# ChuhanZhou/News_Recommendation_Model

Hardware: AMD Instinct MI355X
Metric: train impressions/sec (higher is better)
Workload: dtype f32

## Files before the change

news_recommendation_model_amd/csrc/frontend.hip:

```cpp
#include <algorithm>
#include "common.hpp"
#include "frontend.hpp"

namespace nrm {

template <typename XT>
__device__ __forceinline__ int row_index(const XT* xr, int col, int limit, int* err) {
    const int i = (int)xr[col];
    if (i < 0 || i >= limit) { *err = 1; return i < 0 ? 0 : limit - 1; }
    return i;
}

constexpr int FE_MAXSUB = 16;
constexpr int FE_HDR = 6 + FE_MAXSUB;
struct RowHeaders {
    int* idx;
    float* sen;
};

template <typename XT>
__device__ __forceinline__ void stage_headers(const FrontendParams& p, int xcols, int* err, const XT* __restrict__ x, int r_lo, int nr,
                                              const RowHeaders& hd, int nthreads) {
    const int P = p.P, NS = p.n_sub;
    const int c_cat = 4 + P, c_sub = c_cat + 1, c_sen = c_sub + NS, c_typ = c_sen + 3;
    const int items = 9 + NS;
    for (int i = threadIdx.x; i < nr * items; i += nthreads) {
        const int r = i / items, k = i - r * items;
        const XT* xr = x + (size_t)(r_lo + r) * xcols;
        if (k < 4) {
            const int lim = k == 0 ? p.n_year : k == 1 ? p.n_month : k == 2 ? p.n_day : p.n_hour;
            hd.idx[r * FE_HDR + k] = row_index(xr, k, lim, err);
        } else if (k == 4) {
            hd.idx[r * FE_HDR + 4] = row_index(xr, c_cat, p.n_cat, err);
        } else if (k == 5) {
            hd.idx[r * FE_HDR + 5] = row_index(xr, c_typ, p.n_type, err);
        } else if (k < 6 + NS) {
            hd.idx[r * FE_HDR + k] = row_index(xr, c_sub + (k - 6), p.n_cat, err);
        } else {
            hd.sen[r * 4 + (k - 6 - NS)] = (float)xr[c_sen + (k - 6 - NS)];
        }
    }
}

constexpr int FWD_ROWS = 8;
constexpr int FE_THREADS = 256;

template <typename XT>
__global__ __launch_bounds__(FE_THREADS) void frontend_fwd_kernel(const FrontendParams p, const XT* __restrict__ x, int nrows) {
    __shared__ int h_idx[FWD_ROWS * FE_HDR];
    __shared__ float h_sen[FWD_ROWS * 4];
    const int r_lo = blockIdx.x * FWD_ROWS, nr = min(FWD_ROWS, nrows - r_lo);
    const RowHeaders hd = {h_idx, h_sen};
    stage_headers(p, p.xcols, p.err, x, r_lo, nr, hd, FE_THREADS);
    __syncthreads();
    const int P = p.P, NS = p.n_sub;
    const int c_beh = 4 + P + 1 + NS + 3 + 1;
    const int e0 = p.e0, e1 = p.e1, e2 = p.e2, e3 = p.e3;
    const int width = e0 + e1 + e2 + e3 + (p.behaviour ? 2 : 0);
    const float inv_ns = 1.0f / (float)NS;
    float* lab = p.lab + (size_t)r_lo * p.ldlab;
    for (int i = threadIdx.x; i < nr * p.ldlab; i += FE_THREADS) {
        const int r = i / p.ldlab, c = i - r * p.ldlab;
        const int* hi = h_idx + r * FE_HDR;
        float v = 0.f;
        if (c < e0) {
            float sub = 0.f;
            for (int k = 0; k < NS; ++k) sub += p.cat_tab[(size_t)hi[6 + k] * e0 + c];
            v = p.cat_tab[(size_t)hi[4] * e0 + c] + sub * inv_ns;
        } else if (c < e0 + e1) {
            const int j = c - e0;
            const float pre = p.sen_b[j] + p.sen_w[j * 3] * h_sen[r * 4] + p.sen_w[j * 3 + 1] * h_sen[r * 4 + 1] + p.sen_w[j * 3 + 2] * h_sen[r * 4 + 2];
            v = fmaxf(pre, 0.f);
        } else if (c < e0 + e1 + e2) {
            v = p.type_tab[(size_t)hi[5] * e2 + (c - e0 - e1)];
        } else if (c < e0 + e1 + e2 + e3) {
            const int k = c - e0 - e1 - e2;
            v = p.year_tab[(size_t)hi[0] * e3 + k] + p.month_tab[(size_t)hi[1] * e3 + k] + p.day_tab[(size_t)hi[2] * e3 + k] + p.hour_tab[(size_t)hi[3] * e3 + k];
        } else if (c < width) {
            v = (float)x[(size_t)(r_lo + r) * p.xcols + c_beh + (c - (e0 + e1 + e2 + e3))];
        }
        lab[i] = v;
    }
    float* ti = p.ti + (size_t)r_lo * p.ldti;
    for (int i = threadIdx.x; i < nr * p.ldti; i += FE_THREADS) {
        const int r = i / p.ldti, c = i - r * p.ldti;
        ti[i] = c < P ? (float)x[(size_t)(r_lo + r) * p.xcols + 4 + c] : 0.f;
    }
}

constexpr int FE_ROWS = 32;
constexpr int FE_MAX_BLOCKS = 512;

template <typename XT>
__global__ __launch_bounds__(FE_THREADS) void frontend_bwd_kernel(const FrontendParams p, const XT* __restrict__ x,
                                                                 const float* __restrict__ dlab, int lddl, int nrows) {
    extern __shared__ float sm[];
    const int e0 = p.e0, e1 = p.e1, e2 = p.e2, e3 = p.e3;
    float* a_type = sm;
    float* a_year = a_type + p.n_type * e2;
    float* a_month = a_year + p.n_year * e3;
    float* a_day = a_month + p.n_month * e3;
    float* a_hour = a_day + p.n_day * e3;
    float* a_sen = a_hour + p.n_hour * e3;
    const int total = (int)(a_sen + e1 * 4 - sm);
    const RowHeaders hd = {reinterpret_cast<int*>(sm + total), sm + total + FE_ROWS * FE_HDR};
    for (int i = threadIdx.x; i < total; i += FE_THREADS) sm[i] = 0.f;
    int dummy = 0;
    const int NS = p.n_sub;
    const float inv_ns = 1.0f / (float)NS;
    const int small = e1 + e2 + e3;
    const int ngroups = (nrows + FE_ROWS - 1) / FE_ROWS;
    for (int grp = blockIdx.x; grp < ngroups; grp += gridDim.x) {
        const int r_lo = grp * FE_ROWS, nr = min(FE_ROWS, nrows - r_lo);
        __syncthreads();
        stage_headers(p, p.xcols, &dummy, x, r_lo, nr, hd, FE_THREADS);
        __syncthreads();
        const float* g0 = dlab + (size_t)r_lo * lddl;
        for (int i = threadIdx.x; i < (p.d_cat_tab ? nr * e0 : 0); i += FE_THREADS) {
            const int r = i / e0, c = i - r * e0;
            const int* hi = hd.idx + r * FE_HDR;
            const float gv = g0[(size_t)r * lddl + c];
            atomicAdd(p.d_cat_tab + (size_t)hi[4] * e0 + c, gv);
            const float gs = gv * inv_ns;
            for (int k = 0; k < NS; ++k) atomicAdd(p.d_cat_tab + (size_t)hi[6 + k] * e0 + c, gs);
        }
        for (int i = threadIdx.x; i < (p.d_type_tab ? nr * small : 0); i += FE_THREADS) {
            const int r = i / small, cs = i - r * small;
            const float gv = g0[(size_t)r * lddl + e0 + cs];
            const int* hi = hd.idx + r * FE_HDR;
            if (cs < e1) {
                const float s0 = hd.sen[r * 4], s1 = hd.sen[r * 4 + 1], s2 = hd.sen[r * 4 + 2];
                const float pre = p.sen_b[cs] + p.sen_w[cs * 3] * s0 + p.sen_w[cs * 3 + 1] * s1 + p.sen_w[cs * 3 + 2] * s2;
                if (pre > 0.f && gv != 0.f) {
                    atomicAdd(a_sen + cs * 4 + 0, gv * s0);
                    atomicAdd(a_sen + cs * 4 + 1, gv * s1);
                    atomicAdd(a_sen + cs * 4 + 2, gv * s2);
                    atomicAdd(a_sen + cs * 4 + 3, gv);
                }
            } else if (cs < e1 + e2) {
                atomicAdd(a_type + hi[5] * e2 + (cs - e1), gv);
            } else {
                const int k = cs - e1 - e2;
                atomicAdd(a_year + hi[0] * e3 + k, gv);
                atomicAdd(a_month + hi[1] * e3 + k, gv);
                atomicAdd(a_day + hi[2] * e3 + k, gv);
                atomicAdd(a_hour + hi[3] * e3 + k, gv);
            }
        }
    }
    __syncthreads();
    if (!p.d_type_tab) return;
    for (int i = threadIdx.x; i < p.n_type * e2; i += FE_THREADS) if (a_type[i] != 0.f) atomicAdd(p.d_type_tab + i, a_type[i]);
    for (int i = threadIdx.x; i < p.n_year * e3; i += FE_THREADS) if (a_year[i] != 0.f) atomicAdd(p.d_year_tab + i, a_year[i]);
    for (int i = threadIdx.x; i < p.n_month * e3; i += FE_THREADS) if (a_month[i] != 0.f) atomicAdd(p.d_month_tab + i, a_month[i]);
    for (int i = threadIdx.x; i < p.n_day * e3; i += FE_THREADS) if (a_day[i] != 0.f) atomicAdd(p.d_day_tab + i, a_day[i]);
    for (int i = threadIdx.x; i < p.n_hour * e3; i += FE_THREADS) if (a_hour[i] != 0.f) atomicAdd(p.d_hour_tab + i, a_hour[i]);
    for (int i = threadIdx.x; i < e1 * 4; i += FE_THREADS) {
        const float v = a_sen[i];
        if (v != 0.f) {
            const int j = i >> 2, w = i & 3;
            if (w < 3) atomicAdd(p.d_sen_w + j * 3 + w, v); else atomicAdd(p.d_sen_b + j, v);
        }
    }
}

static size_t bwd_lds_bytes(const FrontendParams& p) {
    return sizeof(float) * ((size_t)p.n_type * p.e2 + (size_t)(p.n_year + p.n_month + p.n_day + p.n_hour) * p.e3 + (size_t)p.e1 * 4 +
                            (size_t)FE_ROWS * (FE_HDR + 4));
}

hipError_t frontend_fwd_launch(const FrontendParams& p, const void* x, int x_is_f64, int nrows, hipStream_t st) {
    if (nrows <= 0) return hipSuccess;
    if (p.n_sub > FE_MAXSUB) return hipErrorInvalidValue;
    const dim3 grid((nrows + FWD_ROWS - 1) / FWD_ROWS);
    if (x_is_f64) hipLaunchKernelGGL(frontend_fwd_kernel<double>, grid, dim3(FE_THREADS), 0, st, p, (const double*)x, nrows);
    else          hipLaunchKernelGGL(frontend_fwd_kernel<float>, grid, dim3(FE_THREADS), 0, st, p, (const float*)x, nrows);
    return hipGetLastError();
}

hipError_t frontend_bwd_launch(const FrontendParams& p, const void* x, int x_is_f64, const float* dlab, int lddl,
                               int nrows, hipStream_t st) {
    if (nrows <= 0) return hipSuccess;
    const size_t shm = bwd_lds_bytes(p);
    if (shm > 160 * 1024 || p.n_sub > FE_MAXSUB) return hipErrorInvalidValue;
    const dim3 grid(std::min((nrows + FE_ROWS - 1) / FE_ROWS, FE_MAX_BLOCKS));
    if (x_is_f64) {
        if (shm > 64 * 1024) { hipError_t e = hipFuncSetAttribute((const void*)frontend_bwd_kernel<double>, hipFuncAttributeMaxDynamicSharedMemorySize, (int)shm); if (e != hipSuccess) return e; }
        hipLaunchKernelGGL(frontend_bwd_kernel<double>, grid, dim3(FE_THREADS), shm, st, p, (const double*)x, dlab, lddl, nrows);
    } else {
        if (shm > 64 * 1024) { hipError_t e = hipFuncSetAttribute((const void*)frontend_bwd_kernel<float>, hipFuncAttributeMaxDynamicSharedMemorySize, (int)shm); if (e != hipSuccess) return e; }
        hipLaunchKernelGGL(frontend_bwd_kernel<float>, grid, dim3(FE_THREADS), shm, st, p, (const float*)x, dlab, lddl, nrows);
    }
    return hipGetLastError();
}

constexpr int TB_THREADS = 512;
constexpr int TB_WAVES = TB_THREADS / 64;
constexpr int TB_ROWS = 32;
constexpr int TB_MAXT = 16;
constexpr int TB_MAXTILES = TB_WAVES * TB_MAXT;
constexpr int TB_WG_PER_CU = 2;
constexpr int TB_CB = 4;
constexpr int TB_RED_CELLS = 64, TB_RED_SLICES = 16;

struct TabTile {
    short hdr, ibase;
    short coff, ncol;
    int dst;
    short ldr, ldc;
};
struct TabSet { const void* x; const float* dlab; int nrows, xcols, lddl, nchunks; };
struct TabParams {
    FrontendParams p;
    TabSet set[2];
    int ntiles, tiles_per_wave, cells, ldb, chunks_per_wg;
    float* ws;
    TabTile tile[TB_MAXTILES];
};

__device__ __forceinline__ bool fe_finite(float v) { return fabsf(v) <= 3.402823466e+38f; }

template <typename XT, int NT>
__global__ __launch_bounds__(TB_THREADS, TB_WG_PER_CU * TB_WAVES / 4) void tab_grad_kernel(const TabParams q) {
    extern __shared__ float sm[];
    const FrontendParams& p = q.p;
    const int e0 = p.e0, e1 = p.e1, e2 = p.e2, e3 = p.e3;
    const int small = e1 + e2 + e3, ldb = q.ldb;
    float* s_b = sm;
    float* s_wb = s_b + TB_ROWS * ldb;
    float* s_sen = s_wb + 4 * e1;
    float* s_sa = s_sen + TB_ROWS * 4;
    int* s_idx = reinterpret_cast<int*>(s_sa + TB_ROWS * 4);
    const RowHeaders hd = {s_idx, s_sen};
    const int lane = threadIdx.x & 63, wave = __builtin_amdgcn_readfirstlane(threadIdx.x >> 6);
    const int li = lane & 15, lk = lane >> 4;

    for (int i = threadIdx.x; i < e1 * 4; i += TB_THREADS) s_wb[i] = (i & 3) < 3 ? p.sen_w[(i >> 2) * 3 + (i & 3)] : p.sen_b[i >> 2];

    const int t_lo = wave * q.tiles_per_wave;
    const int my_nt = max(0, min(q.tiles_per_wave, q.ntiles - t_lo));
    int t_desc[NT];
    f32x4 acc[NT];
#pragma unroll
    for (int t = 0; t < NT; ++t) {
        const TabTile& d = q.tile[min(t_lo + t, TB_MAXTILES - 1)];
        const int v = t < my_nt ? (d.hdr + 1) | (d.ibase << 3) | (d.coff << 18) : 1 | (0x7fff << 3);
        t_desc[t] = __builtin_amdgcn_readfirstlane(v);
        acc[t] = f32x4{0.f, 0.f, 0.f, 0.f};
    }

    int dummy = 0;
    const int nchunks = q.set[0].nchunks + q.set[1].nchunks;
    const int ch_lo = blockIdx.x * q.chunks_per_wg, ch_hi = min(nchunks, ch_lo + q.chunks_per_wg);
    for (int ch = ch_lo; ch < ch_hi; ++ch) {
        const int si = ch >= q.set[0].nchunks;
        const TabSet& set = q.set[si];
        const int r_lo = (ch - (si ? q.set[0].nchunks : 0)) * TB_ROWS, nr = min(TB_ROWS, set.nrows - r_lo);
        const int nr4 = (nr + 3) & ~3;
        const float* g0 = set.dlab + (size_t)r_lo * set.lddl + e0;
        __syncthreads();
        for (int cb = 0; cb < small; cb += 64 * TB_CB) {
            float gvs[TB_ROWS / TB_WAVES][TB_CB];
#pragma unroll
            for (int k = 0; k < TB_ROWS / TB_WAVES; ++k)
#pragma unroll
                for (int u = 0; u < TB_CB; ++u) {
                    const int r = wave + k * TB_WAVES, c = cb + 64 * u + lane;
                    gvs[k][u] = (r < nr && c < small) ? g0[(size_t)r * set.lddl + c] : 0.f;
                }
            if (cb == 0) {
                stage_headers(p, set.xcols, &dummy, reinterpret_cast<const XT*>(set.x), r_lo, nr, hd, TB_THREADS);
                __syncthreads();
                for (int i = threadIdx.x; i < nr4 * 4; i += TB_THREADS) {
                    const int r = i >> 2, k = i & 3;
                    const bool ok = r < nr && fe_finite(s_sen[r * 4]) && fe_finite(s_sen[r * 4 + 1]) && fe_finite(s_sen[r * 4 + 2]);
                    s_sa[i] = ok ? (k < 3 ? s_sen[i] : 1.f) : 0.f;
                }
                for (int i = nr * FE_HDR + threadIdx.x; i < nr4 * FE_HDR; i += TB_THREADS) s_idx[i] = -1;
            }
#pragma unroll
            for (int k = 0; k < TB_ROWS / TB_WAVES; ++k) {
                const int r = wave + k * TB_WAVES;
                if (r >= nr4) break;
                const int* hi = s_idx + r * FE_HDR;
#pragma unroll
                for (int u = 0; u < TB_CB; ++u) {
                    const int c = cb + 64 * u + lane;
                    if (c >= small) break;
                    const float gv = gvs[k][u];
                    float v = 0.f;
                    if (r < nr) {
                        const bool fin = fe_finite(gv);
                        if (c < e1) {
                            const float s0 = s_sen[r * 4], s1 = s_sen[r * 4 + 1], s2 = s_sen[r * 4 + 2];
                            const f32x4 wb = *reinterpret_cast<const f32x4*>(s_wb + 4 * c);
                            const float pre = wb[3] + wb[0] * s0 + wb[1] * s1 + wb[2] * s2;
                            const bool on = pre > 0.f && gv != 0.f;
                            const bool slow = !fin || !(fe_finite(s0) && fe_finite(s1) && fe_finite(s2));
                            if (__ballot(slow)) {
                                if (slow && on) {
                                    atomicAdd(p.d_sen_w + c * 3 + 0, gv * s0);
                                    atomicAdd(p.d_sen_w + c * 3 + 1, gv * s1);
                                    atomicAdd(p.d_sen_w + c * 3 + 2, gv * s2);
                                    atomicAdd(p.d_sen_b + c, gv);
                                }
                            }
                            v = (on && !slow) ? gv : 0.f;
                        } else {
                            if (__ballot(!fin)) {
                                if (!fin) {
                                    if (c < e1 + e2) {
                                        atomicAdd(p.d_type_tab + hi[5] * e2 + (c - e1), gv);
                                    } else {
                                        const int kk = c - e1 - e2;
                                        atomicAdd(p.d_year_tab + hi[0] * e3 + kk, gv);
                                        atomicAdd(p.d_month_tab + hi[1] * e3 + kk, gv);
                                        atomicAdd(p.d_day_tab + hi[2] * e3 + kk, gv);
                                        atomicAdd(p.d_hour_tab + hi[3] * e3 + kk, gv);
                                    }
                                }
                            }
                            v = fin ? gv : 0.f;
                        }
                    }
                    s_b[r * ldb + c] = v;
                }
            }
        }
        __syncthreads();
        const int* s_a = reinterpret_cast<const int*>(s_sa);
        const int a_sen = lk * 4 + (li & 3), a_idx = TB_ROWS * 4 + lk * FE_HDR;
        for (int r0 = 0; r0 < nr4; r0 += 4) {
            float b[NT];
            int raw[NT];
#pragma unroll
            for (int t = 0; t < NT; ++t) {
                int d = t_desc[t];
                asm volatile("" : "+s"(d));
                const int hdr = (d & 7) - 1, coff = d >> 18;
                b[t] = s_b[(r0 + lk) * ldb + coff + li];
                raw[t] = s_a[hdr >= 0 ? r0 * FE_HDR + a_idx + hdr : r0 * 4 + a_sen];
            }
#pragma unroll
            for (int t = 0; t < NT; ++t) {
                int d = t_desc[t];
                asm volatile("" : "+s"(d));
                const int m = (d & 7) ? -1 : 0, ibase = (d >> 3) & 0x7fff;
                const int one_hot = raw[t] == ibase + li ? __float_as_int(1.f) : 0, sen = li < 4 ? raw[t] : 0;
                acc[t] = mfma16(__int_as_float((one_hot & m) | (sen & ~m)), b[t], acc[t]);
            }
        }
    }
    float* part = q.ws + (size_t)blockIdx.x * q.cells;
#pragma unroll
    for (int t = 0; t < NT; ++t) {
        if (t < my_nt) {
            const TabTile& d = q.tile[t_lo + t];
            const int nrow = d.hdr >= 0 ? min(16, (d.hdr == 5 ? p.n_type : d.hdr == 0 ? p.n_year : d.hdr == 1 ? p.n_month : d.hdr == 2 ? p.n_day : p.n_hour) - d.ibase) : 4;
#pragma unroll
            for (int k = 0; k < 4; ++k) {
                const int row = 4 * lk + k;
                if (row < nrow && li < d.ncol) part[d.dst + row * d.ldr + li * d.ldc] = acc[t][k];
            }
        }
    }
}

__global__ __launch_bounds__(TB_RED_CELLS * TB_RED_SLICES) void tab_reduce_kernel(const FrontendParams p, const float* __restrict__ ws, int nparts, int cells) {
    __shared__ float s[TB_RED_SLICES][TB_RED_CELLS];
    const int cl = threadIdx.x & (TB_RED_CELLS - 1), slice = threadIdx.x / TB_RED_CELLS;
    const int cell = blockIdx.x * TB_RED_CELLS + cl;
    const int per = (nparts + TB_RED_SLICES - 1) / TB_RED_SLICES;
    float v = 0.f;
    if (cell < cells) {
        const int g_hi = min(nparts, (slice + 1) * per);
        int g = slice * per;
        for (; g + 8 <= g_hi; g += 8) {
            float t[8];
#pragma unroll
            for (int k = 0; k < 8; ++k) t[k] = ws[(size_t)(g + k) * cells + cell];
#pragma unroll
            for (int k = 0; k < 8; ++k) v += t[k];
        }
        for (; g < g_hi; ++g) v += ws[(size_t)g * cells + cell];
    }
    s[slice][cl] = v;
    __syncthreads();
    if (slice || cell >= cells) return;
    v = s[0][cl];
#pragma unroll
    for (int k = 1; k < TB_RED_SLICES; ++k) v += s[k][cl];
    int i = cell;
    float* dst;
    if (i < p.n_type * p.e2) dst = p.d_type_tab + i;
    else if ((i -= p.n_type * p.e2) < p.n_year * p.e3) dst = p.d_year_tab + i;
    else if ((i -= p.n_year * p.e3) < p.n_month * p.e3) dst = p.d_month_tab + i;
    else if ((i -= p.n_month * p.e3) < p.n_day * p.e3) dst = p.d_day_tab + i;
    else if ((i -= p.n_day * p.e3) < p.n_hour * p.e3) dst = p.d_hour_tab + i;
    else { i -= p.n_hour * p.e3; dst = (i & 3) < 3 ? p.d_sen_w + (i >> 2) * 3 + (i & 3) : p.d_sen_b + (i >> 2); }
    *dst += v;
}

struct TabPlan { int ntiles, cells, ldb; size_t shm; };
static bool tab_plan(const FrontendParams& p, TabPlan* pl) {
    if (p.e1 <= 0 || p.e2 <= 0 || p.e3 <= 0 || p.n_type <= 0 || p.n_year <= 0 || p.n_month <= 0 || p.n_day <= 0 || p.n_hour <= 0) return false;
    const long n_time = (long)p.n_year + p.n_month + p.n_day + p.n_hour;
    if (n_time > 30000 || p.n_type > 30000 || (long)p.e1 + p.e2 + p.e3 > 4096) return false;
    auto up = [](int n) { return (n + 15) / 16; };
    const long tiles = (long)up(p.e1) + (long)up(p.n_type) * up(p.e2) +
                       (long)(up(p.n_year) + up(p.n_month) + up(p.n_day) + up(p.n_hour)) * up(p.e3);
    if (tiles > TB_MAXTILES) return false;
    const int small = p.e1 + p.e2 + p.e3;
    pl->ntiles = (int)tiles;
    pl->cells = p.n_type * p.e2 + (int)n_time * p.e3 + 4 * p.e1;
    pl->ldb = (small + 63) / 64 * 64 + 16;
    pl->shm = sizeof(float) * ((size_t)TB_ROWS * pl->ldb + 4 * (size_t)p.e1 + (size_t)TB_ROWS * (8 + FE_HDR));
    return pl->shm <= 64 * 1024;
}

static void tab_grid(long nrows0, long nrows1, int* grid, int* chunks_per_wg) {
    const long nchunks = (nrows0 + TB_ROWS - 1) / TB_ROWS + (nrows1 + TB_ROWS - 1) / TB_ROWS;
    const long cap = (long)TB_WG_PER_CU * device_cus();
    const long per = std::max<long>(1, (nchunks + cap - 1) / cap);
    *chunks_per_wg = (int)per;
    *grid = (int)((nchunks + per - 1) / per);
}

long tab_grad_ws_floats(const FrontendParams& p, long nrows_total) {
    TabPlan pl;
    if (nrows_total <= 0 || nrows_total >= (1L << 31) - 2 * TB_ROWS || p.n_sub > FE_MAXSUB || !tab_plan(p, &pl)) return 0;
    const long nchunks = (nrows_total + TB_ROWS - 1) / TB_ROWS + 1;
    return std::min<long>(nchunks, (long)TB_WG_PER_CU * device_cus()) * pl.cells;
}

hipError_t tab_grad_launch(const FrontendParams& p, const void* x0, int nrows0, int xcols0, const float* dlab0, int lddl0,
                           const void* x1, int nrows1, int xcols1, const float* dlab1, int lddl1, int x_is_f64, float* ws, hipStream_t st) {
    if ((long)nrows0 + nrows1 <= 0) return hipSuccess;
    TabParams q = {};
    TabPlan pl;
    if (p.n_sub > FE_MAXSUB || !tab_plan(p, &pl)) return hipErrorInvalidValue;
    q.p = p;
    q.set[0] = {x0, dlab0, nrows0, xcols0, lddl0, (nrows0 + TB_ROWS - 1) / TB_ROWS};
    q.set[1] = {x1, dlab1, nrows1, xcols1, lddl1, (nrows1 + TB_ROWS - 1) / TB_ROWS};
    q.ntiles = pl.ntiles; q.cells = pl.cells; q.ldb = pl.ldb; q.ws = ws;
    q.tiles_per_wave = (pl.ntiles + TB_WAVES - 1) / TB_WAVES;
    int grid = 0;
    tab_grid(nrows0, nrows1, &grid, &q.chunks_per_wg);
    int nt = 0, cell = 0;
    auto table = [&](int hdr, int n, int e, int coff) {
        for (int ib = 0; ib < n; ib += 16)
            for (int c = 0; c < e; c += 16)
                q.tile[nt++] = {(short)hdr, (short)ib, (short)(coff + c), (short)std::min(16, e - c), cell + ib * e + c, (short)e, 1};
        cell += n * e;
    };
    table(5, p.n_type, p.e2, p.e1);
    table(0, p.n_year, p.e3, p.e1 + p.e2);
    table(1, p.n_month, p.e3, p.e1 + p.e2);
    table(2, p.n_day, p.e3, p.e1 + p.e2);
    table(3, p.n_hour, p.e3, p.e1 + p.e2);
    for (int c = 0; c < p.e1; c += 16) q.tile[nt++] = {-1, 0, (short)c, (short)std::min(16, p.e1 - c), cell + 4 * c, 1, 4};
    if (nt != pl.ntiles || cell + 4 * p.e1 != pl.cells) return hipErrorInvalidValue;
    auto launch = [&](auto kernel) { hipLaunchKernelGGL(kernel, dim3(grid), dim3(TB_THREADS), pl.shm, st, q); };
    if (q.tiles_per_wave <= 4)      x_is_f64 ? launch(tab_grad_kernel<double, 4>) : launch(tab_grad_kernel<float, 4>);
    else if (q.tiles_per_wave <= 8) x_is_f64 ? launch(tab_grad_kernel<double, 8>) : launch(tab_grad_kernel<float, 8>);
    else                            x_is_f64 ? launch(tab_grad_kernel<double, TB_MAXT>) : launch(tab_grad_kernel<float, TB_MAXT>);
    hipLaunchKernelGGL(tab_reduce_kernel, dim3((pl.cells + TB_RED_CELLS - 1) / TB_RED_CELLS), dim3(TB_RED_CELLS * TB_RED_SLICES), 0, st, p, ws, grid, pl.cells);
    return hipGetLastError();
}

struct CatRefs {
    const void* x[2]; const float* dlab[2];
    int nrows[2], xcols[2], lddl[2];
    int c_cat, NS, n_cat, e0;
    long nref;
};

template <typename XT>
// ... 226 lines not shown
```

news_recommendation_model_amd/csrc/gemm.hip:

```cpp
#include <cstdlib>
#include <type_traits>
#include "common.hpp"
#include "gemm.hpp"
#ifndef NRM_PRIO
#define NRM_PRIO 0
#endif
#ifndef NRM_DIAG_GEMM
#define NRM_DIAG_GEMM 0
#endif

namespace nrm {

__global__ void pack_rows_kernel(const float* __restrict__ src, long rs, long cs, int nrows, int ncols,
                                 int rows, int kchunks, float* __restrict__ packed) {
    const long total = (long)kchunks * rows * 16;
    for (long i = (long)blockIdx.x * blockDim.x + threadIdx.x; i < total; i += (long)gridDim.x * blockDim.x) {
        const int j = (int)(i & 15);
        const long rc = i >> 4;
        const int row = (int)(rc % rows);
        const int c = (int)(rc / rows);
        const int slot = (j >> 2) ^ swz4(row);
        const int col = c * 16 + 4 * slot + (j & 3);
        packed[i] = (row < nrows && col < ncols) ? src[row * rs + col * cs] : 0.0f;
    }
// ... 166 lines not shown
        }
        if (!(NRM_DIAG_GEMM & 1)) __syncthreads();
    }
    if (NRM_PRIO) __builtin_amdgcn_s_setprio(0);
    if (NRM_DIAG_GEMM & 2) return;

#pragma unroll
    for (int it = 0; it < NT; ++it) {
        if (it < nt_valid) {
        const int n = n0 + it * 16 + 4 * q;
        const int nb = (n0 + it * 16) * 4;
        f32x4 bb = f32x4{0.f, 0.f, 0.f, 0.f};
        if (EPI != EPI_DGELU && p.bias) {
            bb = __builtin_bit_cast(f32x4, __builtin_amdgcn_raw_buffer_load_b128(rs_b, 16 * q, nb, 0));
#pragma unroll
            for (int e = 0; e < 4; ++e) bb[e] = n + e < p.N ? bb[e] : 0.f;
        }
#pragma unroll
        for (int jt = 0; jt < MT; ++jt) {
            const int rl = (wave * MT + jt) * 16 + r16;
            f32x4 v = acc[it][jt] + bb;
            if (EPI == EPI_BIAS) {
                if (n < p.ldy) store_b128_guarded(__builtin_bit_cast(u32x4, v), rs_y, (unsigned)(rl * p.ldy + 4 * q) * 4u, nb);
            } else if (EPI == EPI_GELU) {
                if (n < p.ldz) store_b128_guarded(__builtin_bit_cast(u32x4, v), rs_z, (unsigned)(rl * p.ldz + 4 * q) * 4u, nb);
                const f32x4 g = gelu4(v);
                if (n < p.ldy) store_b128_guarded(__builtin_bit_cast(u32x4, g), rs_y, (unsigned)(rl * p.ldy + 4 * q) * 4u, nb);
            } else if (EPI == EPI_MUL) {
                if (n < p.ldz) store_b128_guarded(__builtin_bit_cast(u32x4, v), rs_z, (unsigned)(rl * p.ldz + 4 * q) * 4u, nb);
                f32x4 mm = f32x4{0.f, 0.f, 0.f, 0.f};
                if (n < p.ldm) mm = __builtin_bit_cast(f32x4, __builtin_amdgcn_raw_buffer_load_b128(rs_m, (unsigned)(rl * p.ldm + 4 * q) * 4u, nb, 0));
                if (n < p.ldy) store_b128_guarded(__builtin_bit_cast(u32x4, v * mm), rs_y, (unsigned)(rl * p.ldy + 4 * q) * 4u, nb);
            } else {
                f32x4 zz = f32x4{0.f, 0.f, 0.f, 0.f};
                if (n < p.ldz) zz = __builtin_bit_cast(f32x4, __builtin_amdgcn_raw_buffer_load_b128(rs_z, (unsigned)(rl * p.ldz + 4 * q) * 4u, nb, 0));
                const f32x4 g = gelu_grad4_times(zz, acc[it][jt]);
                if (n < p.ldy) store_b128_guarded(__builtin_bit_cast(u32x4, g), rs_y, (unsigned)(rl * p.ldy + 4 * q) * 4u, nb);
            }
        }
        }
        __builtin_amdgcn_sched_barrier(0);
    }
#endif
}

GemmNtPlan gemm_nt_plan(int N) {
    const int n16 = (N + 15) / 16;
    GemmNtPlan pl;
    if (n16 <= 4) { pl.NT = 4; pl.MT = 4; }
    else {
        const int p13 = (n16 + 12) / 13 * 13, p8 = (n16 + 7) / 8 * 8;
        int best = p13 <= p8 ? p13 : p8;
        if (p13 <= p8) { pl.NT = 13; pl.MT = 1; } else { pl.NT = 8; pl.MT = 3; }
        static const bool narrow = [] { const char* e = getenv("NRM_NT_NARROW"); return !(e && e[0] == '0'); }();
        const int p9 = (n16 + 8) / 9 * 9, p5 = (n16 + 4) / 5 * 5;
        if (narrow && p9 * 10 <= best * 9) { pl.NT = 9; pl.MT = 2; best = p9; }
        if (narrow && p5 * 10 <= best * 9) { pl.NT = 5; pl.MT = 4; best = p5; }
    }
    pl.nchunks = (n16 + pl.NT - 1) / pl.NT;
    pl.rows = pl.nchunks * pl.NT * 16;
    return pl;
}

template <int NT, int MT, int WPE = 2, int KC = 1>
static hipError_t launch_nt(const GemmNtParams& p, const GemmNtPlan& pl, int epi, hipStream_t st) {
    constexpr int BM = 4 * MT * 16;
    const dim3 grid((p.M + BM - 1) / BM, pl.nchunks), block(256);
    if (KC > 1) {
        constexpr int lds = 2 * KC * (NT * 16 + BM) * 16 * 4;
        static_assert(lds <= 160 * 1024, "two stages must fit the CU's LDS");
    }
    switch (epi) {
        case EPI_BIAS:  hipLaunchKernelGGL((gemm_nt_kernel<NT, MT, EPI_BIAS, WPE, KC>), grid, block, 0, st, p); break;
        case EPI_GELU:  hipLaunchKernelGGL((gemm_nt_kernel<NT, MT, EPI_GELU, WPE, KC>), grid, block, 0, st, p); break;
        case EPI_DGELU: hipLaunchKernelGGL((gemm_nt_kernel<NT, MT, EPI_DGELU, WPE, KC>), grid, block, 0, st, p); break;
        case EPI_MUL:   hipLaunchKernelGGL((gemm_nt_kernel<NT, MT, EPI_MUL, WPE, KC>), grid, block, 0, st, p); break;
        default: return hipErrorInvalidValue;
    }
    return hipGetLastError();
}

hipError_t gemm_nt_launch(const GemmNtParams& p, const GemmNtPlan& pl, int epi, hipStream_t st) {
    if (p.M <= 0) return hipSuccess;
    static const bool small_m = [] { const char* e = getenv("NRM_NT_SMALLM"); return !(e && e[0] == '0'); }();
    const long wgs = (long)((p.M + 64 * pl.MT - 1) / (64 * pl.MT)) * pl.nchunks;
    const char* kc_e = getenv("NRM_NT_KC");
    int kc = kc_e ? atoi(kc_e) : 1;
    if (kc != 2 && kc != 4) kc = 1;
    if (p.kchunks < 2 * kc) kc = p.kchunks >= 4 ? 2 : 1;
    if (kc > 1 && (pl.MT == 1 || (small_m && wgs < 512))) {
        if (kc == 4) {
            if (pl.NT == 4) return launch_nt<4, 1, 1, 4>(p, pl, epi, st);
            if (pl.NT == 5) return launch_nt<5, 1, 1, 4>(p, pl, epi, st);
            if (pl.NT == 8) return launch_nt<8, 1, 1, 4>(p, pl, epi, st);
            if (pl.NT == 9) return launch_nt<9, 1, 1, 4>(p, pl, epi, st);
            if (pl.NT == 13) return launch_nt<13, 1, 1, 4>(p, pl, epi, st);
        } else {
            if (pl.NT == 4) return launch_nt<4, 1, 2, 2>(p, pl, epi, st);
            if (pl.NT == 5) return launch_nt<5, 1, 2, 2>(p, pl, epi, st);
            if (pl.NT == 8) return launch_nt<8, 1, 2, 2>(p, pl, epi, st);
            if (pl.NT == 9) return launch_nt<9, 1, 2, 2>(p, pl, epi, st);
            if (pl.NT == 13) return launch_nt<13, 1, 2, 2>(p, pl, epi, st);
        }
    }
    if (small_m && pl.MT > 1 && wgs < 512) {
        if (pl.NT == 4) return launch_nt<4, 1, 4>(p, pl, epi, st);
        if (pl.NT == 5) return launch_nt<5, 1, 4>(p, pl, epi, st);
        if (pl.NT == 8) return launch_nt<8, 1, 4>(p, pl, epi, st);
        if (pl.NT == 9) return launch_nt<9, 1, 4>(p, pl, epi, st);
    }
    if (pl.NT == 4) return launch_nt<4, 4>(p, pl, epi, st);
    if (pl.NT == 5) return launch_nt<5, 4>(p, pl, epi, st);
    if (pl.NT == 8) return launch_nt<8, 3>(p, pl, epi, st);
    if (pl.NT == 9) return launch_nt<9, 2, 3>(p, pl, epi, st);
    static const int use13x2 = [] { const char* e = getenv("NRM_NT_13X2"); return e && e[0] == '1' ? 1 : 0; }();
    if (use13x2) return launch_nt<13, 2>(p, pl, epi, st);
    return launch_nt<13, 1, 4>(p, pl, epi, st);
}

template <int W> __device__ __forceinline__ int tn_col(int t, int r) {
    if (W == 2) return 2 * r + t;
    if (W == 5 && t == 4) return 64 + r;
    if (W == 8 && t >= 4) return 64 + 4 * r + (t - 4);
    return 4 * r + t;
}
#if defined(__HIP_DEVICE_COMPILE__)
template <int W> __device__ __forceinline__ void tn_load(float (&v)[W], const __amdgpu_buffer_rsrc_t rs, unsigned vlo, unsigned vhi, int soff) {
    if constexpr (W == 2) {
        const auto x = __builtin_amdgcn_raw_buffer_load_b64(rs, vlo, soff, 0);
        v[0] = __uint_as_float(x[0]); v[1] = __uint_as_float(x[1]);
    } else {
        const u32x4 x = __builtin_amdgcn_raw_buffer_load_b128(rs, vlo, soff, 0);
#pragma unroll
        for (int e = 0; e < 4; ++e) v[e] = __uint_as_float(x[e]);
        if constexpr (W == 5) v[4] = __uint_as_float(__builtin_amdgcn_raw_buffer_load_b32(rs, vhi, soff, 0));
        if constexpr (W == 8) {
            const u32x4 y = __builtin_amdgcn_raw_buffer_load_b128(rs, vhi, soff, 0);
#pragma unroll
            for (int e = 0; e < 4; ++e) v[4 + e] = __uint_as_float(y[e]);
        }
    }
}
#endif
constexpr int tn_waves_per_simd(int KT, int DT) { return KT * DT <= 16 ? 4 : 3; }

template <int KT, int DT>
__global__ __launch_bounds__(256, tn_waves_per_simd(KT, DT)) void gemm_tn_kernel(const GemmTnParams p) {
#if defined(__HIP_DEVICE_COMPILE__)
    const int tid = threadIdx.x;
    const int lane = tid & 63;
    const int wave = __builtin_amdgcn_readfirstlane(tid >> 6);
    const int r16 = lane & 15, q = lane >> 4;
    const int nblk = gridDim.x * gridDim.y, lin = blockIdx.y * gridDim.x + blockIdx.x;
    const int xq = nblk >> 3, xr = nblk & 7, xcd = lin & 7;
    const int logical = (xcd < xr ? xcd * (xq + 1) : xr * (xq + 1) + (xcd - xr) * xq) + (lin >> 3);
    const int bx = logical % gridDim.x, by = logical / gridDim.x;
    const int ti = bx % p.nti, tj = bx / p.nti;
    const int i0 = ti * (KT * 16), j0 = tj * (DT * 16);
    if (p.zero_out) {
        const long n4 = p.zero_n >> 2;
        const f32x4 z4 = f32x4{0.f, 0.f, 0.f, 0.f};
        for (long i = (long)lin * 256 + tid; i < n4; i += (long)nblk * 256) reinterpret_cast<f32x4*>(p.zero_out)[i] = z4;
        for (long i = (n4 << 2) + (long)lin * 256 + tid; i < p.zero_n; i += (long)nblk * 256) p.zero_out[i] = 0.f;
    }
    const int split = by * 4 + wave;
    if (split >= p.nsplit) return;
    const int r_lo = split * p.rps;
    const int r_hi = min(p.R, r_lo + p.rps);
    const int nrows = r_hi - r_lo;
    const int nsteps = nrows > 0 ? (nrows + 3) >> 2 : 0;

    const __amdgpu_buffer_rsrc_t ra = __builtin_amdgcn_make_buffer_rsrc(
        const_cast<float*>(p.A) + (size_t)r_lo * p.lda, 0, nrows > 0 ? ((nrows - 1) * p.lda + p.acols) * 4 : 0, 0x00020000);
    const __amdgpu_buffer_rsrc_t rb = __builtin_amdgcn_make_buffer_rsrc(
        const_cast<float*>(p.B) + (size_t)r_lo * p.ldb, 0, nrows > 0 ? ((nrows - 1) * p.ldb + p.bcols) * 4 : 0, 0x00020000);
    const unsigned va_lo = (unsigned)(q * p.lda + i0 + tn_col<KT>(0, r16)) * 4u, va_hi = (unsigned)(q * p.lda + i0 + tn_col<KT>(KT - 1, r16) - (KT == 8 ? 3 : 0)) * 4u;
    const unsigned vb_lo = (unsigned)(q * p.ldb + j0 + tn_col<DT>(0, r16)) * 4u, vb_hi = (unsigned)(q * p.ldb + j0 + tn_col<DT>(DT - 1, r16) - (DT == 8 ? 3 : 0)) * 4u;
    const int astep = p.lda * 16, bstep = p.ldb * 16;

    f32x4 C[KT][DT];
    float cs[KT];
#pragma unroll
    for (int it = 0; it < KT; ++it) cs[it] = 0.f;

    float a0[KT], b0[DT], a1[KT], b1[DT], a2[KT], b2[DT], a3[KT], b3[DT];
    auto load_step = [&](float (&a)[KT], float (&b)[DT], int s) {
        tn_load<KT>(a, ra, va_lo, va_hi, s * astep);
        tn_load<DT>(b, rb, vb_lo, vb_hi, s * bstep);
    };
    auto mfma_batch = [&](const float (&a)[KT], const float (&b)[DT]) {
#pragma unroll
        for (int it = 0; it < KT; ++it) {
            cs[it] += a[it];
#pragma unroll
            for (int jt = 0; jt < DT; ++jt) C[it][jt] = mfma16(a[it], b[jt], C[it][jt]);
        }
    };
#pragma unroll
    for (int it = 0; it < KT; ++it)
#pragma unroll
        for (int jt = 0; jt < DT; ++jt) C[it][jt] = f32x4{0.f, 0.f, 0.f, 0.f};
    if (0 < nsteps) load_step(a0, b0, 0);
    if (1 < nsteps) load_step(a1, b1, 1);
    if (2 < nsteps) load_step(a2, b2, 2);
    for (int s = 0; s < nsteps; s += 4) {
        if (NRM_DIAG_GEMM & 8) { mfma_batch(a0, b0); mfma_batch(a1, b1); mfma_batch(a2, b2); mfma_batch(a0, b0); continue; }
        if (s + 3 < nsteps) load_step(a3, b3, s + 3);
        mfma_batch(a0, b0);
        if (s + 1 < nsteps) {
            if (s + 4 < nsteps) load_step(a0, b0, s + 4);
            mfma_batch(a1, b1);
        }
        if (s + 2 < nsteps) {
            if (s + 5 < nsteps) load_step(a1, b1, s + 5);
            mfma_batch(a2, b2);
        }
        if (s + 3 < nsteps) {
            if (s + 6 < nsteps) load_step(a2, b2, s + 6);
            mfma_batch(a3, b3);
        }
    }

    float* wsp = p.ws + (size_t)split * p.ncols_j * p.ldws;
#pragma unroll
    for (int jt = 0; jt < DT; ++jt) {
        const int j = j0 + tn_col<DT>(jt, r16);
        if (j >= p.ncols_j) continue;
        float* row = wsp + (size_t)j * p.ldws + i0;
        if constexpr (KT == 2) {
#pragma unroll
            for (int h = 0; h < 2; ++h) {
                const int ii = 8 * q + 4 * h;
                if (i0 + ii < p.ldws) *reinterpret_cast<f32x4*>(row + ii) = f32x4{C[0][jt][2 * h], C[1][jt][2 * h], C[0][jt][2 * h + 1], C[1][jt][2 * h + 1]};
            }
        } else {
#pragma unroll
            for (int g = 0; g < (KT == 8 ? 2 : 1); ++g)
#pragma unroll
                for (int e = 0; e < 4; ++e) {
                    const int ii = 64 * g + 16 * q + 4 * e;
                    if (i0 + ii < p.ldws)
                        *reinterpret_cast<f32x4*>(row + ii) = f32x4{C[4 * g][jt][e], C[4 * g + 1][jt][e], C[4 * g + 2][jt][e], C[4 * g + 3][jt][e]};
                }
            if constexpr (KT == 5)
                if (i0 + 64 + 4 * q < p.ldws) *reinterpret_cast<f32x4*>(row + 64 + 4 * q) = C[KT - 1][jt];
        }
    }
    if (p.colsum && tj == 0) {
#pragma unroll
        for (int it = 0; it < KT; ++it) {
            const float v = sum_rows4(cs[it]);
            const int i = i0 + tn_col<KT>(it, r16);
            if (q == 0 && i < p.ldws) p.colsum[(size_t)split * p.ldws + i] = v;
        }
    }
#endif
}

static const int kTnShapes[][2] = {{4, 4}, {5, 5}, {2, 8}, {8, 2}, {5, 2}, {2, 5}};

GemmTnPlan gemm_tn_plan(int ncols_i, int ncols_j, int R, int target_waves, int mma) {
    GemmTnPlan pl;
    const int ni16 = (ncols_i + 15) / 16, nj16 = (ncols_j + 15) / 16;
    pl.KT = pl.DT = 4;
    long best = -1;
    static const bool wide = [] { const char* e = getenv("NRM_TN_SHAPES"); return !(e && e[0] == '0'); }();
    for (int k = 0; k < (mma ? 1 : (wide ? 6 : 2)); ++k) {
        const int kt = kTnShapes[k][0], dt = kTnShapes[k][1];
        const long w = (long)((ni16 + kt - 1) / kt) * kt * ((nj16 + dt - 1) / dt) * dt;
        if (best < 0 || w < best) { best = w; pl.KT = kt; pl.DT = dt; }
    }
    pl.nti = (ni16 + pl.KT - 1) / pl.KT;
    pl.ntj = (nj16 + pl.DT - 1) / pl.DT;
    const int tiles = pl.nti * pl.ntj;
    if (target_waves <= 0) target_waves = 1024 * (mma ? 1 : tn_waves_per_simd(pl.KT, pl.DT));
    int ns = target_waves / tiles / 4 * 4;
    if (ns < 4) ns = 4;
    const int max_ns = (R + 127) / 128;
    if (ns > max_ns) ns = max_ns < 1 ? 1 : max_ns;
    pl.rps = ((R + ns - 1) / ns + 3) / 4 * 4;
    if (mma) pl.rps = (pl.rps + 31) / 32 * 32;
    if (pl.rps < 4) pl.rps = 4;
    pl.nsplit = (R + pl.rps - 1) / pl.rps;
    if (pl.nsplit < 1) pl.nsplit = 1;
    return pl;
}

hipError_t gemm_tn_launch(GemmTnParams p, const GemmTnPlan& pl, hipStream_t st) {
    p.nti = pl.nti; p.nsplit = pl.nsplit; p.rps = pl.rps;
    const dim3 grid(pl.nti * pl.ntj, (pl.nsplit + 3) / 4), block(256);
    const int shape = pl.KT * 16 + pl.DT;
    switch (shape) {
        case 4 * 16 + 4: hipLaunchKernelGGL((gemm_tn_kernel<4, 4>), grid, block, 0, st, p); break;
        case 5 * 16 + 5: hipLaunchKernelGGL((gemm_tn_kernel<5, 5>), grid, block, 0, st, p); break;
        case 2 * 16 + 8: hipLaunchKernelGGL((gemm_tn_kernel<2, 8>), grid, block, 0, st, p); break;
        case 8 * 16 + 2: hipLaunchKernelGGL((gemm_tn_kernel<8, 2>), grid, block, 0, st, p); break;
        case 5 * 16 + 2: hipLaunchKernelGGL((gemm_tn_kernel<5, 2>), grid, block, 0, st, p); break;
        case 2 * 16 + 5: hipLaunchKernelGGL((gemm_tn_kernel<2, 5>), grid, block, 0, st, p); break;
        default: return hipErrorInvalidValue;
    }
    return hipGetLastError();
}

__device__ __forceinline__ void slab_reduce_block(const SlabReduceParams& p, int spc, int bx, int by, int nby,
                                                  float (*tile)[129]) {
    const int tx = threadIdx.x, ty = threadIdx.y;
    const int nbi = (p.ni + 127) / 128;
    if (by == nby - 1) {
        if (!p.vec) return;
        const int i = bx * 256 + ty * 32 + tx;
        if (i < p.ni) {
            float a = 0.f;
#pragma unroll 8
            for (int s = 0; s < p.nsplit; ++s) a += p.vec[(size_t)s * p.ldws + i];
            p.vec_out[i] = a;
        }
        return;
    }
    if (bx >= nbi * ((p.nj + 31) / 32)) return;
    const int i0 = (bx % nbi) * 128, j0 = (bx / nbi) * 32;
    const int s_lo = by * spc, s_hi = min(p.nsplit, s_lo + spc);
    const size_t slab = (size_t)p.nj * p.ldws;
    f32x4 a[4];
#pragma unroll
    for (int r = 0; r < 4; ++r) a[r] = f32x4{0.f, 0.f, 0.f, 0.f};
    const int i = i0 + 4 * tx;
    if (i < p.ldws) {
#pragma unroll 4
        for (int s = s_lo; s < s_hi; ++s) {
            const float* src = p.ws + s * slab + (size_t)(j0 + ty) * p.ldws + i;
#pragma unroll
            for (int r = 0; r < 4; ++r)
                if (j0 + ty + 8 * r < p.nj) a[r] += *reinterpret_cast<const f32x4*>(src + (size_t)8 * r * p.ldws);
        }
    }
#pragma unroll
    for (int r = 0; r < 4; ++r)
#pragma unroll
        for (int e = 0; e < 4; ++e) tile[ty + 8 * r][4 * tx + e] = a[r][e];
    __syncthreads();
    const int t = ty * 32 + tx, jj = t & 31;
    const int j = j0 + jj;
    if (j < p.nj) {
        for (int il = t >> 5; il < 128; il += 8) {
            const int ii = i0 + il;
            if (ii >= p.ni) break;
            const float v = tile[jj][il];
            atomicAdd(p.out + ii * p.ors + j * p.ocs, v);
            if (p.out2) atomicAdd(p.out2 + ii * p.ors2 + j * p.ocs2, p.sign2 * v);
        }
    }
}

__global__ __launch_bounds__(256) void slab_reduce_kernel(const SlabReduceParams p, int spc) {
    __shared__ float tile[32][129];
    slab_reduce_block(p, spc, blockIdx.x, blockIdx.y, gridDim.y, tile);
}

__global__ __launch_bounds__(256) void slab_reduce_multi_kernel(const SlabTable tab) {
    __shared__ float tile[32][129];
    int b = blockIdx.x, e = 0;
    while (e + 1 < tab.n && b >= tab.first[e + 1]) ++e;
    b -= tab.first[e];
    slab_reduce_block(tab.e[e], tab.spc[e], b % tab.gx[e], b / tab.gx[e], tab.nchunk[e] + 1, tile);
}

static void slab_plan(const SlabReduceParams& p, int& gx, int& nchunk, int& spc) {
    const int nbi = (p.ni + 127) / 128, nbj = (p.nj + 31) / 32;
    const int tiles = nbi * nbj;
    gx = tiles;
    if (p.vec && (p.ni + 255) / 256 > gx) gx = (p.ni + 255) / 256;
    nchunk = 512 / tiles;
    if (nchunk > 128) nchunk = 128;
    if (nchunk > (p.nsplit + 3) / 4) nchunk = (p.nsplit + 3) / 4;
    if (nchunk < 1) nchunk = 1;
    spc = (p.nsplit + nchunk - 1) / nchunk;
    nchunk = (p.nsplit + spc - 1) / spc;
}

hipError_t slab_reduce_launch(const SlabReduceParams& p, hipStream_t st) {
    if (p.ni <= 0 || p.nj <= 0) return hipSuccess;
    int gx, nchunk, spc;
    slab_plan(p, gx, nchunk, spc);
    hipLaunchKernelGGL(slab_reduce_kernel, dim3(gx, nchunk + 1), dim3(32, 8), 0, st, p, spc);
    return hipGetLastError();
}

hipError_t slab_reduce_multi_launch(const SlabReduceParams* ps, int n, hipStream_t st) {
    for (int base = 0; base < n; base += SLAB_MAX) {
        SlabTable tab;
        const int m = n - base < SLAB_MAX ? n - base : SLAB_MAX;
        int blocks = 0;
        for (int e = 0; e < m; ++e) {
            tab.e[e] = ps[base + e];
            slab_plan(tab.e[e], tab.gx[e], tab.nchunk[e], tab.spc[e]);
            tab.first[e] = blocks;
            blocks += tab.gx[e] * (tab.nchunk[e] + 1);
        }
        tab.n = m;
        hipLaunchKernelGGL(slab_reduce_multi_kernel, dim3(blocks), dim3(32, 8), 0, st, tab);
        const hipError_t err = hipGetLastError();
        if (err != hipSuccess) return err;
    }
    return hipSuccess;
}

int gemm_diag_flags() { return NRM_DIAG_GEMM ? 0x100 : 0; }

}
```

Before: 35650.

## Add vectorized wide frontend forward kernel and group split-K slab reduction in-block

Adds a new forward frontend kernel that assigns 32 threads per row and uses vector loads and stores for the input copy and the embedding-table label assembly. It is enabled by default when the pointers are aligned. Separately, the slab reduction now runs four split groups per block (1024 threads) with a swizzled shared-memory partial buffer, summing partials in LDS before the atomics. This is meant to cut per-element memory transactions and the number of global atomics, at the cost of larger blocks, more shared memory, and a changed chunk planning heuristic.

```diff
diff --git a/news_recommendation_model_amd/csrc/frontend.hip b/news_recommendation_model_amd/csrc/frontend.hip
--- a/news_recommendation_model_amd/csrc/frontend.hip
+++ b/news_recommendation_model_amd/csrc/frontend.hip
@@ -1,4 +1,6 @@
 #include <algorithm>
+#include <cstdint>
+#include <cstdlib>
 #include "common.hpp"
 #include "frontend.hpp"
 
@@ -88,6 +90,154 @@
     }
 }
 
+template <typename XT>
+__device__ __forceinline__ float fwd_label_elem(const FrontendParams& p, const XT* __restrict__ xr, const int* hi, const float* hs, int c,
+                                                float inv_ns, int c_beh, int width) {
+    const int NS = p.n_sub, e0 = p.e0, e1 = p.e1, e2 = p.e2, e3 = p.e3;
+    float v = 0.f;
+    if (c < e0) {
+        float sub = 0.f;
+        for (int k = 0; k < NS; ++k) sub += p.cat_tab[(size_t)hi[6 + k] * e0 + c];
+        v = p.cat_tab[(size_t)hi[4] * e0 + c] + sub * inv_ns;
+    } else if (c < e0 + e1) {
+        const int j = c - e0;
+        const float pre = p.sen_b[j] + p.sen_w[j * 3] * hs[0] + p.sen_w[j * 3 + 1] * hs[1] + p.sen_w[j * 3 + 2] * hs[2];
+        v = fmaxf(pre, 0.f);
+    } else if (c < e0 + e1 + e2) {
+        v = p.type_tab[(size_t)hi[5] * e2 + (c - e0 - e1)];
+    } else if (c < e0 + e1 + e2 + e3) {
+        const int k = c - e0 - e1 - e2;
+        v = p.year_tab[(size_t)hi[0] * e3 + k] + p.month_tab[(size_t)hi[1] * e3 + k] + p.day_tab[(size_t)hi[2] * e3 + k] + p.hour_tab[(size_t)hi[3] * e3 + k];
+    } else if (c < width) {
+        v = (float)xr[c_beh + (c - (e0 + e1 + e2 + e3))];
+    }
+    return v;
+}
+
+template <typename XT, int V>
+__global__ __launch_bounds__(FE_THREADS) void frontend_fwd_wide_kernel(const FrontendParams p, const XT* __restrict__ x, int nrows) {
+    static_assert(FWD_ROWS * 32 == FE_THREADS, "32 threads per row");
+    __shared__ int h_idx[FWD_ROWS * FE_HDR];
+    __shared__ float h_sen[FWD_ROWS * 4];
+    const int r_lo = blockIdx.x * FWD_ROWS, nr = min(FWD_ROWS, nrows - r_lo);
+    const RowHeaders hd = {h_idx, h_sen};
+    const int r = threadIdx.x >> 5, q0 = threadIdx.x & 31;
+    const bool live = r < nr;
+    const XT* xr = x + (size_t)(r_lo + (live ? r : 0)) * p.xcols;
+    using XV = __attribute__((ext_vector_type(V))) XT;
+    using FV = __attribute__((ext_vector_type(V))) float;
+    constexpr int FWD_CB = 4;
+    XT in[FWD_CB][V];
+    auto request = [&](int c0) {
+#pragma unroll
+        for (int u = 0; u < FWD_CB; ++u) {
+            const int c = c0 + V * (q0 + 32 * u);
+            if (live && c < p.P) {
+                if constexpr (V == 1) {
+                    in[u][0] = xr[4 + c];
+                } else {
+                    const XV t = *reinterpret_cast<const XV*>(xr + 4 + c);
+#pragma unroll
+                    for (int e = 0; e < V; ++e) in[u][e] = t[e];
+                }
+            }
+        }
+    };
+    auto deliver = [&](int c0, float* ti) {
+#pragma unroll
+        for (int u = 0; u < FWD_CB; ++u) {
+            const int c = c0 + V * (q0 + 32 * u);
+            if (c < p.ldti) {
+                FV o;
+#pragma unroll
+                for (int e = 0; e < V; ++e) o[e] = c + e < p.P ? (float)in[u][e] : 0.f;
+                if constexpr (V == 1) ti[c] = o[0]; else *reinterpret_cast<FV*>(ti + c) = o;
+            }
+        }
+    };
+    request(0);
+    stage_headers(p, p.xcols, p.err, x, r_lo, nr, hd, FE_THREADS);
+    __syncthreads();
+    if (!live) return;
+    {
+        float* ti = p.ti + (size_t)(r_lo + r) * p.ldti;
+        deliver(0, ti);
+        for (int c0 = V * 32 * FWD_CB; c0 < p.ldti; c0 += V * 32 * FWD_CB) {
+            request(c0);
+            deliver(c0, ti);
+        }
+    }
+    const int P = p.P, NS = p.n_sub;
+    const int c_beh = 4 + P + 1 + NS + 3 + 1;
+    const int e0 = p.e0, e1 = p.e1, e2 = p.e2, e3 = p.e3;
+    const int b1 = e0 + e1, b2 = b1 + e2, b3 = b2 + e3;
+    const int width = b3 + (p.behaviour ? 2 : 0);
+    const bool vec0 = (e0 & 3) == 0, vec2 = ((e2 | b1) & 3) == 0, vec3 = ((e3 | b2) & 3) == 0;
+    const float inv_ns = 1.0f / (float)NS;
+    const int* hi = h_idx + r * FE_HDR;
+    const float* hs = h_sen + r * 4;
+    float* lab = p.lab + (size_t)(r_lo + r) * p.ldlab;
+    for (int c = 4 * q0; c < p.ldlab; c += 4 * 32) {
+        f32x4 v;
+        if (vec0 && c + 4 <= e0) {
+            const f32x4 cat = *reinterpret_cast<const f32x4*>(p.cat_tab + (size_t)hi[4] * e0 + c);
+            f32x4 sub = {0.f, 0.f, 0.f, 0.f};
+            for (int k0 = 0; k0 < NS; k0 += 8) {
+                f32x4 t[8];
+#pragma unroll
+                for (int k = 0; k < 8; ++k)
+                    if (k0 + k < NS) t[k] = *reinterpret_cast<const f32x4*>(p.cat_tab + (size_t)hi[6 + k0 + k] * e0 + c);
+#pragma unroll
+                for (int k = 0; k < 8; ++k)
+                    if (k0 + k < NS) sub += t[k];
+            }
+#pragma unroll
+            for (int e = 0; e < 4; ++e) v[e] = cat[e] + sub[e] * inv_ns;
+        } else if (vec2 && c >= b1 && c + 4 <= b2) {
+            v = *reinterpret_cast<const f32x4*>(p.type_tab + (size_t)hi[5] * e2 + (c - b1));
+        } else if (vec3 && c >= b2 && c + 4 <= b3) {
+            const int k = c - b2;
+            const f32x4 ty = *reinterpret_cast<const f32x4*>(p.year_tab + (size_t)hi[0] * e3 + k);
+            const f32x4 tm = *reinterpret_cast<const f32x4*>(p.month_tab + (size_t)hi[1] * e3 + k);
+            const f32x4 td = *reinterpret_cast<const f32x4*>(p.day_tab + (size_t)hi[2] * e3 + k);
+            const f32x4 th = *reinterpret_cast<const f32x4*>(p.hour_tab + (size_t)hi[3] * e3 + k);
+#pragma unroll
+            for (int e = 0; e < 4; ++e) v[e] = ty[e] + tm[e] + td[e] + th[e];
+        } else if (c >= e0 && c + 4 <= b1) {
+            const int j = c - e0;
+            float b[4], w[4][3];
+#pragma unroll
+            for (int e = 0; e < 4; ++e) {
+                b[e] = p.sen_b[j + e];
+#pragma unroll
+                for (int k = 0; k < 3; ++k) w[e][k] = p.sen_w[(j + e) * 3 + k];
+            }
+#pragma unroll
+            for (int e = 0; e < 4; ++e) {
+                const float pre = b[e] + w[e][0] * hs[0] + w[e][1] * hs[1] + w[e][2] * hs[2];
+                v[e] = fmaxf(pre, 0.f);
+            }
+        } else if (c >= b1 && c + 4 <= b2) {
+            const float* row = p.type_tab + (size_t)hi[5] * e2 + (c - b1);
+#pragma unroll
+            for (int e = 0; e < 4; ++e) v[e] = row[e];
+        } else if (c >= b2 && c + 4 <= b3) {
+            const int k = c - b2;
+            const float *ry = p.year_tab + (size_t)hi[0] * e3 + k, *rm = p.month_tab + (size_t)hi[1] * e3 + k;
+            const float *rd = p.day_tab + (size_t)hi[2] * e3 + k, *rh = p.hour_tab + (size_t)hi[3] * e3 + k;
+            float ty[4], tm[4], td[4], th[4];
+#pragma unroll
+            for (int e = 0; e < 4; ++e) { ty[e] = ry[e]; tm[e] = rm[e]; td[e] = rd[e]; th[e] = rh[e]; }
+#pragma unroll
+            for (int e = 0; e < 4; ++e) v[e] = ty[e] + tm[e] + td[e] + th[e];
+        } else {
+#pragma unroll
+            for (int e = 0; e < 4; ++e) v[e] = fwd_label_elem(p, xr, hi, hs, c + e, inv_ns, c_beh, width);
+        }
+        *reinterpret_cast<f32x4*>(lab + c) = v;
+    }
+}
+
 constexpr int FE_ROWS = 32;
 constexpr int FE_MAX_BLOCKS = 512;
 
@@ -173,6 +323,24 @@
     if (nrows <= 0) return hipSuccess;
     if (p.n_sub > FE_MAXSUB) return hipErrorInvalidValue;
     const dim3 grid((nrows + FWD_ROWS - 1) / FWD_ROWS);
+    auto al16 = [](const void* q) { return (reinterpret_cast<uintptr_t>(q) & 15) == 0; };
+    const char* knob = getenv("NRM_FE_FWD_WIDE");
+    const bool wide = !(knob && knob[0] == '0') && (p.ldlab & 3) == 0 && al16(x) && al16(p.lab) && al16(p.ti) && al16(p.cat_tab) &&
+                      al16(p.type_tab) && al16(p.year_tab) && al16(p.month_tab) && al16(p.day_tab) && al16(p.hour_tab);
+    if (wide) {
+        const int row_bytes = p.xcols * (x_is_f64 ? 8 : 4);
+        int v = (row_bytes % 16 == 0 ? 16 : row_bytes % 8 == 0 ? 8 : 4) / (x_is_f64 ? 8 : 4);
+        while (v > 1 && p.ldti % v) v >>= 1;
+        if (x_is_f64) {
+            if (v >= 2) hipLaunchKernelGGL((frontend_fwd_wide_kernel<double, 2>), grid, dim3(FE_THREADS), 0, st, p, (const double*)x, nrows);
+            else        hipLaunchKernelGGL((frontend_fwd_wide_kernel<double, 1>), grid, dim3(FE_THREADS), 0, st, p, (const double*)x, nrows);
+        } else {
+            if (v >= 4)      hipLaunchKernelGGL((frontend_fwd_wide_kernel<float, 4>), grid, dim3(FE_THREADS), 0, st, p, (const float*)x, nrows);
+            else if (v >= 2) hipLaunchKernelGGL((frontend_fwd_wide_kernel<float, 2>), grid, dim3(FE_THREADS), 0, st, p, (const float*)x, nrows);
+            else             hipLaunchKernelGGL((frontend_fwd_wide_kernel<float, 1>), grid, dim3(FE_THREADS), 0, st, p, (const float*)x, nrows);
+        }
+        return hipGetLastError();
+    }
     if (x_is_f64) hipLaunchKernelGGL(frontend_fwd_kernel<double>, grid, dim3(FE_THREADS), 0, st, p, (const double*)x, nrows);
     else          hipLaunchKernelGGL(frontend_fwd_kernel<float>, grid, dim3(FE_THREADS), 0, st, p, (const float*)x, nrows);
     return hipGetLastError();
diff --git a/news_recommendation_model_amd/csrc/gemm.hip b/news_recommendation_model_amd/csrc/gemm.hip
--- a/news_recommendation_model_amd/csrc/gemm.hip
+++ b/news_recommendation_model_amd/csrc/gemm.hip
@@ -492,12 +492,13 @@
     return hipGetLastError();
 }
 
-__device__ __forceinline__ void slab_reduce_block(const SlabReduceParams& p, int spc, int bx, int by, int nby,
-                                                  float (*tile)[129]) {
-    const int tx = threadIdx.x, ty = threadIdx.y;
+constexpr int SLAB_GROUPS = 4;
+__device__ __forceinline__ void slab_reduce_block(const SlabReduceParams& p, int spc, int nchunk, int bx, int by, int nby,
+                                                  float (*part)[32][128]) {
+    const int tx = threadIdx.x, ty = threadIdx.y, grp = threadIdx.z;
     const int nbi = (p.ni + 127) / 128;
     if (by == nby - 1) {
-        if (!p.vec) return;
+        if (!p.vec || grp) return;
         const int i = bx * 256 + ty * 32 + tx;
         if (i < p.ni) {
             float a = 0.f;
@@ -509,50 +510,57 @@
     }
     if (bx >= nbi * ((p.nj + 31) / 32)) return;
     const int i0 = (bx % nbi) * 128, j0 = (bx / nbi) * 32;
-    const int s_lo = by * spc, s_hi = min(p.nsplit, s_lo + spc);
-    const size_t slab = (size_t)p.nj * p.ldws;
-    f32x4 a[4];
-#pragma unroll
-    for (int r = 0; r < 4; ++r) a[r] = f32x4{0.f, 0.f, 0.f, 0.f};
-    const int i = i0 + 4 * tx;
-    if (i < p.ldws) {
-#pragma unroll 4
-        for (int s = s_lo; s < s_hi; ++s) {
-            const float* src = p.ws + s * slab + (size_t)(j0 + ty) * p.ldws + i;
-#pragma unroll
-            for (int r = 0; r < 4; ++r)
-                if (j0 + ty + 8 * r < p.nj) a[r] += *reinterpret_cast<const f32x4*>(src + (size_t)8 * r * p.ldws);
-        }
-    }
-#pragma unroll
-    for (int r = 0; r < 4; ++r)
-#pragma unroll
-        for (int e = 0; e < 4; ++e) tile[ty + 8 * r][4 * tx + e] = a[r][e];
+    const int ng = min(SLAB_GROUPS, nchunk - by * SLAB_GROUPS);
+    if (grp < ng) {
+        const int s_lo = (by * SLAB_GROUPS + grp) * spc, s_hi = min(p.nsplit, s_lo + spc);
+        const size_t slab = (size_t)p.nj * p.ldws;
+        f32x4 a[4];
+#pragma unroll
+        for (int r = 0; r < 4; ++r) a[r] = f32x4{0.f, 0.f, 0.f, 0.f};
+        const int i = i0 + 4 * tx;
+        if (i < p.ldws) {
+#pragma unroll 2
+            for (int s = s_lo; s < s_hi; ++s) {
+                const float* src = p.ws + s * slab + (size_t)(j0 + ty) * p.ldws + i;
+#pragma unroll
+                for (int r = 0; r < 4; ++r)
+                    if (j0 + ty + 8 * r < p.nj) a[r] += *reinterpret_cast<const f32x4*>(src + (size_t)8 * r * p.ldws);
+            }
+        }
+#pragma unroll
+        for (int r = 0; r < 4; ++r) {
+            const int jl = ty + 8 * r;
+            *reinterpret_cast<f32x4*>(&part[grp][jl][4 * (tx ^ jl)]) = a[r];
+        }
+    }
     __syncthreads();
-    const int t = ty * 32 + tx, jj = t & 31;
+    const int t = (grp * 8 + ty) * 32 + tx, jj = t & 31;
     const int j = j0 + jj;
     if (j < p.nj) {
-        for (int il = t >> 5; il < 128; il += 8) {
+        for (int il = t >> 5; il < 128; il += 8 * SLAB_GROUPS) {
             const int ii = i0 + il;
             if (ii >= p.ni) break;
-            const float v = tile[jj][il];
+            const int c = 4 * ((il >> 2) ^ jj) + (il & 3);
+            float v = part[0][jj][c];
+            for (int g = 1; g < ng; ++g) v += part[g][jj][c];
             atomicAdd(p.out + ii * p.ors + j * p.ocs, v);
             if (p.out2) atomicAdd(p.out2 + ii * p.ors2 + j * p.ocs2, p.sign2 * v);
         }
     }
 }
 
-__global__ __launch_bounds__(256) void slab_reduce_kernel(const SlabReduceParams p, int spc) {
-    __shared__ float tile[32][129];
-    slab_reduce_block(p, spc, blockIdx.x, blockIdx.y, gridDim.y, tile);
-}
-
-__global__ __launch_bounds__(256) void slab_reduce_multi_kernel(const SlabTable tab) {
-    __shared__ float tile[32][129];
+__global__ __launch_bounds__(256 * SLAB_GROUPS, 8) void slab_reduce_kernel(const SlabReduceParams p, int spc, int nchunk) {
+    __shared__ float part[SLAB_GROUPS][32][128];
+    slab_reduce_block(p, spc, nchunk, blockIdx.x, blockIdx.y, gridDim.y, part);
+}
+
+__global__ __launch_bounds__(256 * SLAB_GROUPS, 8) void slab_reduce_multi_kernel(const SlabTable tab) {
+    __shared__ float part[SLAB_GROUPS][32][128];
     int b = blockIdx.x, e = 0;
     while (e + 1 < tab.n && b >= tab.first[e + 1]) ++e;
     b -= tab.first[e];
-    slab_reduce_block(tab.e[e], tab.spc[e], b % tab.gx[e], b / tab.gx[e], tab.nchunk[e] + 1, tile);
+    const int nwg = (tab.nchunk[e] + SLAB_GROUPS - 1) / SLAB_GROUPS;
+    slab_reduce_block(tab.e[e], tab.spc[e], tab.nchunk[e], b % tab.gx[e], b / tab.gx[e], nwg + 1, part);
 }
 
 static void slab_plan(const SlabReduceParams& p, int& gx, int& nchunk, int& spc) {
@@ -562,7 +570,9 @@
     if (p.vec && (p.ni + 255) / 256 > gx) gx = (p.ni + 255) / 256;
     nchunk = 512 / tiles;
     if (nchunk > 128) nchunk = 128;
-    if (nchunk > (p.nsplit + 3) / 4) nchunk = (p.nsplit + 3) / 4;
+    nchunk = (nchunk + SLAB_GROUPS - 1) / SLAB_GROUPS * SLAB_GROUPS;
+    const int most = nchunk > SLAB_GROUPS ? (p.nsplit + 3) / 4 : (p.nsplit + 1) / 2;
+    if (nchunk > most) nchunk = most;
     if (nchunk < 1) nchunk = 1;
     spc = (p.nsplit + nchunk - 1) / nchunk;
     nchunk = (p.nsplit + spc - 1) / spc;
@@ -572,7 +582,8 @@
     if (p.ni <= 0 || p.nj <= 0) return hipSuccess;
     int gx, nchunk, spc;
     slab_plan(p, gx, nchunk, spc);
-    hipLaunchKernelGGL(slab_reduce_kernel, dim3(gx, nchunk + 1), dim3(32, 8), 0, st, p, spc);
+    const int nwg = (nchunk + SLAB_GROUPS - 1) / SLAB_GROUPS;
+    hipLaunchKernelGGL(slab_reduce_kernel, dim3(gx, nwg + 1), dim3(32, 8, SLAB_GROUPS), 0, st, p, spc, nchunk);
     return hipGetLastError();
 }
 
@@ -585,10 +596,10 @@
             tab.e[e] = ps[base + e];
             slab_plan(tab.e[e], tab.gx[e], tab.nchunk[e], tab.spc[e]);
             tab.first[e] = blocks;
-            blocks += tab.gx[e] * (tab.nchunk[e] + 1);
+            blocks += tab.gx[e] * ((tab.nchunk[e] + SLAB_GROUPS - 1) / SLAB_GROUPS + 1);
         }
         tab.n = m;
-        hipLaunchKernelGGL(slab_reduce_multi_kernel, dim3(blocks), dim3(32, 8), 0, st, tab);
+        hipLaunchKernelGGL(slab_reduce_multi_kernel, dim3(blocks), dim3(32, 8, SLAB_GROUPS), 0, st, tab);
         const hipError_t err = hipGetLastError();
         if (err != hipSuccess) return err;
     }
```

Result: no change. 35810, median of 6 (+0.5%).
